# AlvinYH/Faster-VoxelPose

Hardware: AMD Instinct MI355X
Metric: frames/sec at 5-view 80x80x20 voxel (heatmaps -> 3D joints); MPJPE vs ref (mm) in mpjpe_vs_ref_mm (higher is better)
Workload: dtype f32

## Files before the change

faster-voxelpose_amd/csrc/fvp_project.hip:

```cpp
#include <hip/hip_runtime.h>

#include <cstdlib>

#include "fvp_common.h"
#include "fvp_geom.h"

namespace fvp {

template <int NV>
__global__ void __launch_bounds__(256) k_heat_to_cl(const float* __restrict__ heat, float* __restrict__ cl,
                                                    int J, int HW) {
  const int pix = blockIdx.x * 256 + threadIdx.x;
  const size_t bv = blockIdx.y;
  if (pix >= HW) return;
  const float* src = heat + bv * size_t(J) * HW + pix;
  float v[4 * NV];
#pragma unroll
  for (int j = 0; j < 4 * NV; ++j) v[j] = (j < J) ? src[size_t(j) * HW] : 0.0f;
  float4* dst = reinterpret_cast<float4*>(cl + (bv * HW + pix) * size_t(4 * NV));
#pragma unroll
  for (int q = 0; q < NV; ++q) dst[q] = make_float4(v[4 * q], v[4 * q + 1], v[4 * q + 2], v[4 * q + 3]);
}

__global__ void __launch_bounds__(256) k_sample_grid(const float* __restrict__ ax, const float* __restrict__ ay,
                                                     const float* __restrict__ az, int nx, int ny, int nz,
                                                     const Cam* __restrict__ cams, FvpGeom g,
                                                     float* __restrict__ grid) {
  const int n = nx * ny * nz;
  const int i = blockIdx.x * 256 + threadIdx.x;
  const int v = blockIdx.y;
  if (i >= n) return;
  const int iz = i % nz, iy = (i / nz) % ny, ix = i / (nz * ny);
  float gx, gy;
  project_norm(cams[v], g, ax[ix], ay[iy], az[iz], gx, gy);
  grid[(size_t(v) * n + i) * 2 + 0] = gx;
  grid[(size_t(v) * n + i) * 2 + 1] = gy;
}

template <int NV>
__device__ __forceinline__ void backproject_point(const float* __restrict__ heat_cl_frame,
                                                  const Cam* __restrict__ cams, const FvpGeom& g, float wx,
                                                  float wy, float wz, float (&acc)[4 * NV]) {
  const size_t view_stride = size_t(g.H) * g.W * (4 * NV);
  for (int v = 0; v < g.V; ++v) {
    float gx, gy;
    project_norm(cams[v], g, wx, wy, wz, gx, gy);
    const Taps t = bilinear_taps(gx, gy, g.W, g.H);
    float s[4 * NV];
    if (t.inside) {
      sample_view<NV>(heat_cl_frame + v * view_stride, t, s);
    } else {
#pragma unroll
      for (int c = 0; c < 4 * NV; ++c) s[c] = 0.0f;
    }
#pragma unroll
    for (int c = 0; c < 4 * NV; ++c) acc[c] = (v == 0) ? s[c] : __fadd_rn(acc[c], s[c]);
  }
  const float nv = float(g.V);
#pragma unroll
  for (int c = 0; c < 4 * NV; ++c) acc[c] = clampf(__fdiv_rn(acc[c], nv), 0.0f, 1.0f);
}

template <int NV>
__global__ void __launch_bounds__(256)
k_project_whole(const float* __restrict__ heat_cl, const Cam* __restrict__ cams, const int* __restrict__ frame_set,
                const float* __restrict__ ax, const float* __restrict__ ay, const float* __restrict__ az, int X,
                int Y, int Z, FvpGeom g, float* __restrict__ cubes, float* __restrict__ zmax) {
  __shared__ float sm[4 * NV][256];
  const int cpb = 256 / Z;
  const int b = blockIdx.y;
  const int t = threadIdx.x;
  const int cl_ = t / Z, z = t - cl_ * Z;
  const int col = blockIdx.x * cpb + cl_;
  const int ncol = X * Y;
  const bool active = cl_ < cpb && col < ncol;
  const int J = g.J;
  float acc[4 * NV];
#pragma unroll
  for (int c = 0; c < 4 * NV; ++c) acc[c] = 0.0f;
  if (active) {
    const int x = col / Y, y = col - x * Y;
    const float* frame = heat_cl + size_t(b) * g.V * g.H * g.W * (4 * NV);
    backproject_point<NV>(frame, cams + size_t(frame_set[b]) * g.V, g, ax[x], ay[y], az[z], acc);
    if (cubes) {
// ... 613 lines not shown
  if (nP == 0) return 0;
  ProfScope ps(FVP_K_OTHER, as_stream(s));
  const int per = (C * C + 255) / 256;
  const dim3 grid(J, nP);
  const size_t lds = size_t(C) * (C + 1) * sizeof(float);
#define FVP_TRIMAX(PER_) hipLaunchKernelGGL(k_triplane_max<PER_>, grid, dim3(256), lds, as_stream(s), cubes, planes, J, C)
  if (per <= 1) FVP_TRIMAX(1);
  else if (per <= 4) FVP_TRIMAX(4);
  else if (per <= 16) FVP_TRIMAX(16);
  else FVP_TRIMAX(64);
#undef FVP_TRIMAX
  return launch_status();
}

extern "C" int fvp_project_individual_triplane(const float* heat_cl, const float* cams, const int32_t* frame_set,
                                               const int32_t* person_frame, const uint8_t* person_valid,
                                               const int32_t* boxes, const float* fx, const float* fy,
                                               const float* fz, const int32_t* fine, int C, int nP, const FvpGeom* g,
                                               float* planes, int persons_per_frame, const float* fine_grid,
                                               fvp_stream_t s) {
  FVP_REQUIRE(heat_cl && cams && frame_set && person_frame && boxes && fx && fy && fz && planes && nP >= 0);
  FVP_REQUIRE(!fine_grid || fine);
  if (int e = check_geom(g)) return e;
  if (int e = check_cube(C)) return e;
  if (nP == 0) return 0;
  const int ppf = (persons_per_frame > 0 && nP % persons_per_frame == 0) ? persons_per_frame : nP;
  [[maybe_unused]] const int chunks = ceil_div(C * C, 256);
  const int nvl = ceil_div(g->JP, 16);
  ProfScope ps(FVP_K_PROJECT_TRIPLANE, as_stream(s));
  const int F0 = fine_grid ? fine[0] : 0, F1 = fine_grid ? fine[1] : 0, F2 = fine_grid ? fine[2] : 0;
  const int nby = ceil_div(C, kBY);
#if FVP_DIAG
  const int nbx = ceil_div(C, kBX);
  static const bool gather = fvp::diag_env("FVP_TRIPLANE_GATHER") != nullptr;
  const bool quad_form = fvp::diag_env("FVP_TRIPLANE_QUAD") != nullptr;
  static const int tri_ablate_env = fvp::diag_env("FVP_TRI_ABLATE") ? atoi(fvp::diag_env("FVP_TRI_ABLATE")) : 0;
  const char* tt_env = fvp::diag_env("FVP_TRI_TWO_TILE");
  const bool staged = fvp::diag_env("FVP_TRIPLANE_STAGED") != nullptr;
  const bool force_lane = fvp::diag_env("FVP_TRIPLANE_LANE") != nullptr;
  const bool lane_form = !gather && !quad_form && g->JP <= 20 && ((staged && g->JP != 16) || force_lane);
  const int tri_ablate = (tri_ablate_env & ~16) | ((tt_env ? atoi(tt_env) != 0 : lane_form) ? 16 : 0);
  auto cap_lim = [](int cap) { const char* e = fvp::diag_env("FVP_TRI_CAP_PX"); const int v = e ? atoi(e) : cap; return v > 0 && v < cap ? v : cap; };
  const int cap_px = int((36 * 1024) / (size_t(g->JP) * 4));
  const size_t lds = 2 * size_t(cap_px) * g->JP * 4 + 64;
  if (lane_form) {
    const int lq = (g->JP / 4) | 1;
    const int cap_px = int((36 * 1024) / (size_t(lq) * 16));
    const size_t lds = 2 * size_t(cap_px) * lq * 16 + 64;
    FVP_LIMIT(size_t(cap_px) * lq * 4 >= size_t(kBX * kBY + (kBX + kBY) * 32) * g->JP);
#define CALL2(NQ_, CACHED_)                                                                                       \
  {                                                                                                                \
    static LdsOptIn optin;                                                                                         \
    auto k = &k_project_triplane_lds2<NQ_, CACHED_>;                                                              \
    if (int e = lds_opt_in(optin, reinterpret_cast<const void*>(k), lds)) return e;                                \
    hipLaunchKernelGGL(k, dim3(nbx * nby * nP), dim3(kTriThreads), lds, as_stream(s), heat_cl,                     \
                       reinterpret_cast<const Cam*>(cams), frame_set, person_frame, person_valid, boxes, fx, fy, fz, C, \
                       nP, nbx, nby, ppf, cap_px, *g, fine_grid, F0, F1, F2, planes, tri_ablate, cap_lim(cap_px));                  \
  }
#define CASE2(NQ_) case NQ_: if (fine_grid) CALL2(NQ_, true) else CALL2(NQ_, false) break;
    switch (g->JP / 4) {
      CASE2(1) CASE2(2) CASE2(3) CASE2(4) CASE2(5)
      default: return FVP_ELIMIT;
    }
#undef CASE2
#undef CALL2
    return launch_status();
  }
  const bool blk_form = !gather && !quad_form && !staged;
#else
  constexpr bool blk_form = true;
#endif
  if (blk_form && nvl <= 2) {
    const int nbx2 = ceil_div(C, kBlkBX);
    const int bz = nvl == 2 ? 16 : kBlkBZ;
    int zsh = 0;
    while ((1 << zsh) < C) ++zsh;
    const size_t lds_z = (size_t(kBlkBX + kBY) << zsh) * (g->JP + 1) * 4;
#if FVP_DIAG
    const char* zr_env = fvp::diag_env("FVP_TRI_ZRES");
    const bool zres = zr_env && atoi(zr_env) != 0 && (1 << zsh) >= bz && lds_z <= kTriZresMaxLds;
#else
    constexpr bool zres = false;
#endif
    const size_t lds_b = zres ? lds_z : size_t(kBlkBX * kBY + (kBlkBX + kBY) * bz) * (g->JP + 1) * 4;
#define CALLB(NVL_, CACHED_, ZRES_)                                                                                          \
  hipLaunchKernelGGL((k_project_triplane_blk<NVL_, CACHED_, ZRES_>), dim3(nbx2 * nby * nP), dim3(kBlkThreads), lds_b,       \
                     as_stream(s), heat_cl, reinterpret_cast<const Cam*>(cams), frame_set, person_frame, person_valid, boxes, \
                     fx, fy, fz, C, nP, nbx2, nby, ppf, *g, fine_grid, F0, F1, F2, planes, zsh)
#if FVP_DIAG
#define CALLB2(NVL_)                                                                     \
  {                                                                                      \
    if (fine_grid) { if (zres) CALLB(NVL_, true, true); else CALLB(NVL_, true, false); } \
    else { if (zres) CALLB(NVL_, false, true); else CALLB(NVL_, false, false); }         \
  }
#else
#define CALLB2(NVL_)                                                                     \
  {                                                                                      \
    if (fine_grid) CALLB(NVL_, true, false); else CALLB(NVL_, false, false);             \
  }
#endif
    const bool q5 = nvl == 2 && g->JP == 20 && !zres && fvp::diag_env("FVP_TRI_NO_Q5") == nullptr;
    if (q5) {
      if (fine_grid)
        hipLaunchKernelGGL((k_project_triplane_blk<2, true, false, true>), dim3(nbx2 * nby * nP), dim3(kBlkThreads), lds_b, as_stream(s),
                           heat_cl, reinterpret_cast<const Cam*>(cams), frame_set, person_frame, person_valid, boxes, fx, fy, fz, C, nP,
                           nbx2, nby, ppf, *g, fine_grid, F0, F1, F2, planes, zsh);
      else
        hipLaunchKernelGGL((k_project_triplane_blk<2, false, false, true>), dim3(nbx2 * nby * nP), dim3(kBlkThreads), lds_b, as_stream(s),
                           heat_cl, reinterpret_cast<const Cam*>(cams), frame_set, person_frame, person_valid, boxes, fx, fy, fz, C, nP,
                           nbx2, nby, ppf, *g, fine_grid, F0, F1, F2, planes, zsh);
    } else if (nvl == 2) CALLB2(2) else CALLB2(1)
#undef CALLB2
#undef CALLB
    return launch_status();
  }
#if FVP_DIAG
  if (!gather && nvl <= 2) {
    FVP_LIMIT(cap_px >= kBX * kBY + (kBX + kBY) * (nvl == 1 ? 32 : 16));
#define CALL(NVL_, CACHED_)                                                                                        \
  {                                                                                                                \
    static LdsOptIn optin;                                                                                         \
    auto k = &k_project_triplane_lds<NVL_, CACHED_>;                                                               \
    if (int e = lds_opt_in(optin, reinterpret_cast<const void*>(k), lds)) return e;                                \
    hipLaunchKernelGGL(k, dim3(nbx * nby * nP), dim3(kTriThreads), lds, as_stream(s), heat_cl,                     \
                       reinterpret_cast<const Cam*>(cams), frame_set, person_frame, person_valid, boxes, fx, fy, fz, C, \
                       nP, nbx, nby, ppf, cap_px, *g, fine_grid, F0, F1, F2, planes, tri_ablate, cap_lim(cap_px));                  \
  }
    if (nvl == 1) {
      if (fine_grid) CALL(1, true) else CALL(1, false)
    } else {
      if (fine_grid) CALL(2, true) else CALL(2, false)
    }
#undef CALL
    return launch_status();
  }
  if (nvl == 1) {
    auto k = &k_project_triplane<1>;
    hipLaunchKernelGGL(k, dim3(chunks * nP), dim3(1024), 0, as_stream(s), heat_cl, reinterpret_cast<const Cam*>(cams),
                       frame_set, person_frame, person_valid, boxes, fx, fy, fz, C, nP, chunks, ppf, *g, planes);
  } else if (nvl == 2) {
    auto k = &k_project_triplane<2>;
    hipLaunchKernelGGL(k, dim3(chunks * nP), dim3(1024), 0, as_stream(s), heat_cl, reinterpret_cast<const Cam*>(cams),
                       frame_set, person_frame, person_valid, boxes, fx, fy, fz, C, nP, chunks, ppf, *g, planes);
  } else {
    return FVP_ELIMIT;
  }
  return launch_status();
#else
  return FVP_ELIMIT;
#endif
}
```

faster-voxelpose_amd/csrc/fvp_project_lds.h:

```cpp
#pragma once
#include <type_traits>
#include <climits>

namespace fvp {

typedef float f32x2 __attribute__((ext_vector_type(2)));
#ifndef FVP_TRI_PACKED
#define FVP_TRI_PACKED 1
#endif
#ifndef FVP_TRI_EXPLICIT_AS
#define FVP_TRI_EXPLICIT_AS 1
#endif

typedef float f32x4v __attribute__((ext_vector_type(4)));
__device__ __forceinline__ float4 lds_ld4(const float* p) {
  const f32x4v v = *(const __attribute__((address_space(3))) f32x4v*)p;
  return make_float4(v.x, v.y, v.z, v.w);
}
__device__ __forceinline__ float4 glb_ld4(const float* p) {
  const f32x4v v = *(const __attribute__((address_space(1))) f32x4v*)p;
  return make_float4(v.x, v.y, v.z, v.w);
}

struct TapL {
// ... 300 lines not shown
        }
      }
      if (rcur.big) {
        __syncthreads();
        if (v + 1 < V && rnxt.staged) issue_dma(v + 1, rnxt);
      }
      cur = nxt;
      rcur = rnxt;
    }
    __syncthreads();
    if (ablate & 4) continue;
    int* cxy = reinterpret_cast<int*>(smem);
    int* cxz = cxy + kBX * kBY * JP;
    int* cyz = cxz + kBX * BZ * JP;
    const int ncell = (kBX * kBY + (kBX + kBY) * BZ) * JP;
    for (int i = t; i < ncell; i += NT) cxy[i] = 0;
    __syncthreads();
#pragma unroll
    for (int n = 0; n < NVL; ++n)
#pragma unroll
      for (int c = 0; c < 4; ++c) {
        const int ch = 16 * n + 4 * q + c;
        float mz = 0.0f;
#pragma unroll
        for (int i = 0; i < VPT; ++i) {
          const float val = fmaxf(acc[i][n][c], 0.0f);
          mz = fmaxf(mz, val);
          if (val > 0.0f && ch < JP) {
            const int z = zs + 4 * i;
            atomicMax(&cxz[(xx * BZ + z) * JP + ch], __float_as_int(val));
            atomicMax(&cyz[(yy * BZ + z) * JP + ch], __float_as_int(val));
          }
        }
        int mi = __float_as_int(mz);
        mi = imax(mi, dpp_i<0x124>(mi));
        mi = imax(mi, dpp_i<0x128>(mi));
        if (zs == 0 && mi > 0 && ch < JP) cxy[(xx * kBY + yy) * JP + ch] = mi;
      }
    __syncthreads();
    const int lz0 = gz0 - tl2;
    for (int i = t; i < kBX * kBY * J; i += NT) {
      const int ch = i / (kBX * kBY), col = i - ch * (kBX * kBY), cx = col / kBY, cy = col - cx * kBY;
      const int raw = cxy[col * JP + ch];
      if (raw > 0 && gx0 + cx < e0 && gy0 + cy < e1) {
        const int vv = __float_as_int(clampf(__fdiv_rn(__int_as_float(raw), nv), 0.0f, 1.0f));
        if (vv > 0) plane_max(&pxy[size_t(ch) * CC + (gx0 + cx - tl0) * C + (gy0 + cy - tl1)], vv);
      }
    }
    for (int i = t; i < (kBX + kBY) * BZ * J; i += NT) {
      const int ch = i / ((kBX + kBY) * BZ), r = i - ch * ((kBX + kBY) * BZ), a = r / BZ, z = r - a * BZ;
      if (gz0 + z < e2) {
        const int raw = cxz[r * JP + ch];
        const int vv = raw > 0 ? __float_as_int(clampf(__fdiv_rn(__int_as_float(raw), nv), 0.0f, 1.0f)) : 0;
        if (vv > 0) {
          if (a < kBX) {
            if (gx0 + a < e0) plane_max(&pxz[size_t(ch) * CC + (gx0 + a - tl0) * C + lz0 + z], vv);
          } else if (gy0 + a - kBX < e1) {
            plane_max(&pyz[size_t(ch) * CC + (gy0 + a - kBX - tl1) * C + lz0 + z], vv);
          }
        }
      }
    }
    __syncthreads();
  }
}

#endif

#ifndef FVP_TRI_BLK_OCC
#define FVP_TRI_BLK_OCC 4
#endif
#ifndef FVP_TRI_BLK_BX
#define FVP_TRI_BLK_BX 4
#endif
#ifndef FVP_TRI_BLK_BZ
#define FVP_TRI_BLK_BZ 16
#endif
constexpr int kBlkBX = FVP_TRI_BLK_BX, kBlkBZ = FVP_TRI_BLK_BZ;
constexpr int kBlkThreads = kBlkBX * kBY * 4 * 4;
#ifndef FVP_TRI_ZRES_MAX_KB
#define FVP_TRI_ZRES_MAX_KB 48
#endif
constexpr size_t kTriZresMaxLds = size_t(FVP_TRI_ZRES_MAX_KB) * 1024;
template <int NVL, bool CACHED, bool ZRES, bool Q5 = false>
__global__ void __launch_bounds__(kBlkThreads, FVP_TRI_BLK_OCC)
k_project_triplane_blk(const float* __restrict__ heat_cl, const Cam* __restrict__ cams, const int* __restrict__ frame_set,
                       const int* __restrict__ person_frame, const uint8_t* __restrict__ person_valid,
                       const int* __restrict__ boxes, const float* __restrict__ fx, const float* __restrict__ fy,
                       const float* __restrict__ fz, int C, int nP, int nbx, int nby, int ppf, FvpGeom g,
                       const float* __restrict__ fgrid, int F0, int F1, int F2, float* __restrict__ planes, int zsh) {
  static_assert(!Q5 || (NVL == 2 && !ZRES), "the five-quad form replaces the two-group form of the per-z-block kernel");
  constexpr int NVA = Q5 ? 1 : NVL;
  constexpr int BZ = NVL == 1 ? kBlkBZ : 16;
  constexpr int VPT = BZ / 4;
  constexpr int OWN = VPT / 4;
  HIP_DYNAMIC_SHARED(float, smem)
  constexpr int NT = kBlkThreads;
  constexpr int kBX = kBlkBX;
  const int J = g.J, JP = g.JP, CC = C * C, V = g.V, W = g.W, H = g.H;
  int p, blk;
  {
    const int id = blockIdx.x;
    const int bpp = nbx * nby, bpf = ppf * bpp;
    const int nframes = nP / ppf;
    if (nframes % 8 == 0) {
      const int xcd = id & 7, j = id >> 3;
      const int frame = xcd + 8 * (j / bpf), r = j % bpf;
      p = frame * ppf + r / bpp;
      blk = r % bpp;
    } else {
      p = id / bpp;
      blk = id % bpp;
    }
  }
  if (person_valid && !person_valid[p]) return;
  const int* bx = boxes + p * 9;
  const int tl0 = bx[0], tl1 = bx[1], tl2 = bx[2];
  const int s0 = bx[3], s1 = bx[4], s2 = bx[5], e0 = bx[6], e1 = bx[7], e2 = bx[8];
  if (s0 >= e0 || s1 >= e1 || s2 >= e2) return;
  const int xb = blk / nby, yb = blk - xb * nby;
  const int gx0 = s0 + xb * kBX, gy0 = s1 + yb * kBY;
  if (gx0 >= e0 || gy0 >= e1) return;

  const int t = threadIdx.x, q = t & 3;
  const int slot = t >> 2, zs = slot & 3, yy = (slot >> 2) & (kBY - 1), xx = slot / (4 * kBY);
  const int gxi = gx0 + xx, gyi = gy0 + yy;
  const bool col_in = gxi < e0 && gyi < e1;
  const int b = person_frame[p];
  const size_t view_stride = size_t(H) * W * JP;
  const float* frame = heat_cl + size_t(b) * V * view_stride;
  const Cam* cm = cams + size_t(frame_set[b]) * V;
  const float wx = col_in ? fx[gxi] : 0.0f, wy = col_in ? fy[gyi] : 0.0f;
  const size_t nfine = size_t(F0) * F1 * F2;
  const float2* gcol = CACHED ? reinterpret_cast<const float2*>(fgrid) + size_t(frame_set[b]) * V * nfine +
                                    (size_t(col_in ? gxi : 0) * F1 + (col_in ? gyi : 0)) * F2
                              : nullptr;
  float* pxy = planes + (size_t(p) * 3 + 0) * J * CC;
  float* pxz = planes + (size_t(p) * 3 + 1) * J * CC;
  float* pyz = planes + (size_t(p) * 3 + 2) * J * CC;
  const float nv = float(V);
  const int JPp = JP + 1;
  [[maybe_unused]] int mxy[NVL][4];
  [[maybe_unused]] const int zt = 1 << zsh;
  if constexpr (ZRES) {
#pragma unroll
    for (int n = 0; n < NVL; ++n)
#pragma unroll
      for (int c = 0; c < 4; ++c) mxy[n][c] = 0;
    int* cz = reinterpret_cast<int*>(smem);
    const int ncell = ((kBX + kBY) << zsh) * JPp;
    for (int i = t; i < ncell; i += NT) cz[i] = 0;
    __syncthreads();
  }

  for (int gz0 = s2; gz0 < e2; gz0 += BZ) {
    float acc[VPT][NVA][4];
#pragma unroll
    for (int i = 0; i < VPT; ++i)
#pragma unroll
      for (int n = 0; n < NVA; ++n)
#pragma unroll
        for (int c = 0; c < 4; ++c) acc[i][n][c] = 0.0f;
    [[maybe_unused]] float accx[OWN][1][4];
#pragma unroll
    for (int kk = 0; kk < OWN; ++kk)
#pragma unroll
      for (int c = 0; c < 4; ++c) accx[kk][0][c] = 0.0f;
    float2 crd[OWN];
    auto load_coords = [&](int v) {
#pragma unroll
      for (int k = 0; k < OWN; ++k) {
        const int gzi = gz0 + zs + 4 * (q + 4 * k);
        crd[k] = gcol[size_t(v) * nfine + (gzi < F2 ? gzi : F2 - 1)];
      }
    };
    if (CACHED) load_coords(0);
    for (int v = 0; v < V; ++v) {
      TapL mine[OWN];
#pragma unroll
      for (int k = 0; k < OWN; ++k) {
        const int gzi = gz0 + zs + 4 * (q + 4 * k);
        const bool vin = col_in && gzi < e2;
        TapL d;
        d.base = d.dx = d.dy = 0;
        d.w[0] = d.w[1] = d.w[2] = d.w[3] = 0.0f;
        if (vin) {
          float sx, sy;
          if (CACHED) {
            sx = crd[k].x;
            sy = crd[k].y;
          } else {
            project_norm(cm[v], g, wx, wy, fz[gzi], sx, sy);
          }
          int x0, y0, inside;
          float w4[4];
          tap_origin(sx, sy, W, H, x0, y0, w4, inside);
          const int cx0 = imin(imax(x0, 0), W - 1), cx1 = imin(imax(x0 + 1, 0), W - 1);
          const int cy0 = imin(imax(y0, 0), H - 1), cy1 = imin(imax(y0 + 1, 0), H - 1);
          d.base = (cy0 * W + cx0) * JP;
          d.dx = (cx1 - cx0) * JP;
          d.dy = (cy1 - cy0) * W * JP;
#pragma unroll
          for (int c = 0; c < 4; ++c) d.w[c] = ((inside >> c) & 1) ? w4[c] : 0.0f;
        }
        mine[k] = d;
      }
      if (CACHED && v + 1 < V) load_coords(v + 1);
#ifdef FVP_TRI_BLK_NOSAMPLE
      if (mine[0].base != -12345) { acc[0][0][0] += mine[0].w[0] + mine[OWN - 1].w[3] + float(mine[0].base); continue; }
#endif
      const float* gsrc = frame + size_t(v) * view_stride;
      auto sample = [&](const TapL& tv, auto& a, auto own) {
        constexpr bool kOwn = decltype(own)::value;
#pragma unroll
        for (int n = 0; n < (kOwn ? 1 : NVA); ++n) {
          const int ch0 = kOwn ? 16 : 16 * n + 4 * q;
          if (kOwn || ch0 < JP) {
            const float* p0 = gsrc + tv.base + ch0;
            const float4 v0 = glb_ld4(p0), v1 = glb_ld4(p0 + tv.dx), v2 = glb_ld4(p0 + tv.dy), v3 = glb_ld4(p0 + tv.dy + tv.dx);
            const f32x2 w0 = f32x2{tv.w[0], tv.w[0]}, w1 = f32x2{tv.w[1], tv.w[1]}, w2 = f32x2{tv.w[2], tv.w[2]},
                        w3 = f32x2{tv.w[3], tv.w[3]};
            f32x2 lo = f32x2{v0.x, v0.y} * w0, hi = f32x2{v0.z, v0.w} * w0;
            lo = __builtin_elementwise_fma(f32x2{v1.x, v1.y}, w1, lo);
            hi = __builtin_elementwise_fma(f32x2{v1.z, v1.w}, w1, hi);
            lo = __builtin_elementwise_fma(f32x2{v2.x, v2.y}, w2, lo);
            hi = __builtin_elementwise_fma(f32x2{v2.z, v2.w}, w2, hi);
            lo = __builtin_elementwise_fma(f32x2{v3.x, v3.y}, w3, lo);
            hi = __builtin_elementwise_fma(f32x2{v3.z, v3.w}, w3, hi);
            const f32x2 alo = f32x2{a[n][0], a[n][1]} + lo, ahi = f32x2{a[n][2], a[n][3]} + hi;
            a[n][0] = alo.x; a[n][1] = alo.y; a[n][2] = ahi.x; a[n][3] = ahi.y;
          }
        }
      };
#pragma unroll
      for (int k = 0; k < OWN; ++k) {
        { const TapL tv = quad_bcast_l<0>(mine[k]); sample(tv, acc[4 * k + 0], std::false_type{}); }
        { const TapL tv = quad_bcast_l<1>(mine[k]); sample(tv, acc[4 * k + 1], std::false_type{}); }
        { const TapL tv = quad_bcast_l<2>(mine[k]); sample(tv, acc[4 * k + 2], std::false_type{}); }
        { const TapL tv = quad_bcast_l<3>(mine[k]); sample(tv, acc[4 * k + 3], std::false_type{}); }
        if constexpr (Q5) sample(mine[k], accx[k], std::true_type{});
      }
    }
#ifdef FVP_TRI_BLK_NOMAX
    if (acc[0][0][0] != 1.2345e-30f) continue;
#endif
    if constexpr (ZRES) {
      int* rxz = reinterpret_cast<int*>(smem);
      int* ryz = rxz + ((kBX << zsh) * JPp);
      const int zb = gz0 - s2 + zs;
#pragma unroll
      for (int n = 0; n < NVL; ++n)
#pragma unroll
        for (int c = 0; c < 4; ++c) {
          const int ch = 16 * n + 4 * q + c;
          float mz = 0.0f;
#pragma unroll
          for (int i = 0; i < VPT; ++i) {
            const float val = fmaxf(acc[i][n][c], 0.0f);
            mz = fmaxf(mz, val);
            if (val > 0.0f && ch < JP) {
              const int z = zb + 4 * i;
              atomicMax(&rxz[((xx << zsh) + z) * JPp + ch], __float_as_int(val));
              atomicMax(&ryz[((yy << zsh) + z) * JPp + ch], __float_as_int(val));
            }
          }
          int mi = __float_as_int(mz);
          mi = imax(mi, dpp_i<0x124>(mi));
          mi = imax(mi, dpp_i<0x128>(mi));
          mxy[n][c] = imax(mxy[n][c], mi);
        }
      continue;
    }
    int* cxy = reinterpret_cast<int*>(smem);
    int* cxz = cxy + kBX * kBY * JPp;
    int* cyz = cxz + kBX * BZ * JPp;
    const int ncell = (kBX * kBY + (kBX + kBY) * BZ) * JPp;
    __syncthreads();
    for (int i = t; i < ncell; i += NT) cxy[i] = 0;
    __syncthreads();
#pragma unroll
    for (int n = 0; n < NVA; ++n)
#pragma unroll
      for (int c = 0; c < 4; ++c) {
        const int ch = 16 * n + 4 * q + c;
        float mz = 0.0f;
#pragma unroll
        for (int i = 0; i < VPT; ++i) {
          const float val = fmaxf(acc[i][n][c], 0.0f);
          mz = fmaxf(mz, val);
          if (val > 0.0f && ch < JP) {
            const int z = zs + 4 * i;
            atomicMax(&cxz[(xx * BZ + z) * JPp + ch], __float_as_int(val));
            atomicMax(&cyz[(yy * BZ + z) * JPp + ch], __float_as_int(val));
          }
        }
        int mi = __float_as_int(mz);
        mi = imax(mi, dpp_i<0x124>(mi));
        mi = imax(mi, dpp_i<0x128>(mi));
        if (zs == 0 && mi > 0 && ch < JP) cxy[(xx * kBY + yy) * JPp + ch] = mi;
      }
    if constexpr (Q5) {
#pragma unroll
      for (int c = 0; c < 4; ++c) {
        const int ch = 16 + c;
        float mz = 0.0f;
#pragma unroll
        for (int kk = 0; kk < OWN; ++kk) {
          const float val = fmaxf(accx[kk][0][c], 0.0f);
          mz = fmaxf(mz, val);
          if (val > 0.0f) {
            const int z = zs + 4 * (4 * kk + q);
            atomicMax(&cxz[(xx * BZ + z) * JPp + ch], __float_as_int(val));
            atomicMax(&cyz[(yy * BZ + z) * JPp + ch], __float_as_int(val));
          }
        }
        int mi = __float_as_int(mz);
        mi = imax(mi, dpp_i<0x121>(mi));
        mi = imax(mi, dpp_i<0x122>(mi));
        mi = imax(mi, dpp_i<0x124>(mi));
        mi = imax(mi, dpp_i<0x128>(mi));
        if (zs == 0 && q == 0 && mi > 0) cxy[(xx * kBY + yy) * JPp + ch] = mi;
      }
    }
    __syncthreads();
    const int lz0 = gz0 - tl2;
    for (int i = t; i < kBX * kBY * J; i += NT) {
      const int ch = i / (kBX * kBY), col = i - ch * (kBX * kBY), cx = col / kBY, cy = col - cx * kBY;
      const int raw = cxy[col * JPp + ch];
      if (raw > 0 && gx0 + cx < e0 && gy0 + cy < e1) {
        const int vv = __float_as_int(clampf(__fdiv_rn(__int_as_float(raw), nv), 0.0f, 1.0f));
        if (vv > 0) plane_max(&pxy[size_t(ch) * CC + (gx0 + cx - tl0) * C + (gy0 + cy - tl1)], vv);
      }
    }
    for (int i = t; i < (kBX + kBY) * BZ * J; i += NT) {
      const int ch = i / ((kBX + kBY) * BZ), r = i - ch * ((kBX + kBY) * BZ), a = r / BZ, z = r - a * BZ;
      if (gz0 + z < e2) {
        const int raw = cxz[r * JPp + ch];
        const int vv = raw > 0 ? __float_as_int(clampf(__fdiv_rn(__int_as_float(raw), nv), 0.0f, 1.0f)) : 0;
        if (vv > 0) {
          if (a < kBX) {
            if (gx0 + a < e0) plane_max(&pxz[size_t(ch) * CC + (gx0 + a - tl0) * C + lz0 + z], vv);
          } else if (gy0 + a - kBX < e1) {
            plane_max(&pyz[size_t(ch) * CC + (gy0 + a - kBX - tl1) * C + lz0 + z], vv);
          }
        }
      }
    }
  }
  if constexpr (ZRES) {
    __syncthreads();
    if (zs == 0 && col_in) {
#pragma unroll
      for (int n = 0; n < NVL; ++n)
#pragma unroll
        for (int c = 0; c < 4; ++c) {
          const int ch = 16 * n + 4 * q + c;
          if (ch < J && mxy[n][c] > 0) {
            const int vv = __float_as_int(clampf(__fdiv_rn(__int_as_float(mxy[n][c]), nv), 0.0f, 1.0f));
            if (vv > 0) plane_max(&pxy[size_t(ch) * CC + (gxi - tl0) * C + (gyi - tl1)], vv);
          }
        }
    }
    const int* cz = reinterpret_cast<const int*>(smem);
    const int nz = e2 - s2, lz0 = s2 - tl2;
    const int rows = (kBX + kBY) << zsh;
    for (int i = t; i < rows * J; i += NT) {
      static_assert(kBX + kBY == 8, "row count is a power of two");
      const int ch = i >> (zsh + 3), r = i & (rows - 1), a = r >> zsh, z = r & (zt - 1);
      if (z < nz) {
        const int raw = cz[r * JPp + ch];
        const int vv = raw > 0 ? __float_as_int(clampf(__fdiv_rn(__int_as_float(raw), nv), 0.0f, 1.0f)) : 0;
        if (vv > 0) {
          if (a < kBX) {
            if (gx0 + a < e0) plane_max(&pxz[size_t(ch) * CC + (gx0 + a - tl0) * C + lz0 + z], vv);
          } else if (gy0 + a - kBX < e1) {
            plane_max(&pyz[size_t(ch) * CC + (gy0 + a - kBX - tl1) * C + lz0 + z], vv);
          }
        }
      }
    }
  }
}

#if FVP_DIAG
template <int NQ, bool CACHED>
__global__ void __launch_bounds__(kTriThreads, 4)
k_project_triplane_lds2(const float* __restrict__ heat_cl, const Cam* __restrict__ cams, const int* __restrict__ frame_set,
                        const int* __restrict__ person_frame, const uint8_t* __restrict__ person_valid,
                        const int* __restrict__ boxes, const float* __restrict__ fx, const float* __restrict__ fy,
                        const float* __restrict__ fz, int C, int nP, int nbx, int nby, int ppf, int cap_px, FvpGeom g,
                        const float* __restrict__ fgrid, int F0, int F1, int F2, float* __restrict__ planes, int ablate, int cap_lim) {
  constexpr int BZ = 32, VPT = 2, JP = 4 * NQ;
  constexpr int LQ = NQ | 1, LP = 4 * LQ;
  HIP_DYNAMIC_SHARED(float, smem)
  constexpr int NT = kTriThreads;
  const int J = g.J, CC = C * C, V = g.V, W = g.W, H = g.H;
  const int tile_sz = cap_px * LP;
  int* rect = reinterpret_cast<int*>(smem + 2 * size_t(tile_sz));
  int p, blk;
  {
    const int id = blockIdx.x;
    const int bpp = nbx * nby, bpf = ppf * bpp;
    const int nframes = nP / ppf;
    if (nframes % 8 == 0) {
      const int xcd = id & 7, j = id >> 3;
      const int frame = xcd + 8 * (j / bpf), r = j % bpf;
      p = frame * ppf + r / bpp;
      blk = r % bpp;
    } else {
      p = id / bpp;
      blk = id % bpp;
    }
  }
  if (person_valid && !person_valid[p]) return;
  const int* bx = boxes + p * 9;
  const int tl0 = bx[0], tl1 = bx[1], tl2 = bx[2];
  const int s0 = bx[3], s1 = bx[4], s2 = bx[5], e0 = bx[6], e1 = bx[7], e2 = bx[8];
  if (s0 >= e0 || s1 >= e1 || s2 >= e2) return;
  const int xb = blk / nby, yb = blk - xb * nby;
  const int gx0 = s0 + xb * kBX, gy0 = s1 + yb * kBY;
  if (gx0 >= e0 || gy0 >= e1) return;

  const int t = threadIdx.x, lane = t & 63, wave = t >> 6;
  const int z16 = t & 15, yy = (t >> 4) & (kBY - 1), xx = t >> 6;
  const int gxi = gx0 + xx, gyi = gy0 + yy;
  const bool col_in = gxi < e0 && gyi < e1;
  const int b = person_frame[p];
  const size_t view_stride = size_t(H) * W * JP;
  const float* frame = heat_cl + size_t(b) * V * view_stride;
  const Cam* cm = cams + size_t(frame_set[b]) * V;
  const float wx = col_in ? fx[gxi] : 0.0f, wy = col_in ? fy[gyi] : 0.0f;
  const size_t nfine = size_t(F0) * F1 * F2;
  const float2* gcol = CACHED ? reinterpret_cast<const float2*>(fgrid) + size_t(frame_set[b]) * V * nfine +
                                    (size_t(col_in ? gxi : 0) * F1 + (col_in ? gyi : 0)) * F2
                              : nullptr;
  float* pxy = planes + (size_t(p) * 3 + 0) * J * CC;
  float* pxz = planes + (size_t(p) * 3 + 1) * J * CC;
  float* pyz = planes + (size_t(p) * 3 + 2) * J * CC;
  const float nv = float(V);

  struct Own { int xy[VPT]; int inside[VPT]; float w[VPT][4]; };
  float2 crd[VPT];
  auto load_coords = [&](int v, int gz0) {
#pragma unroll
    for (int k = 0; k < VPT; ++k) {
      const int gzi = gz0 + z16 + 16 * k;
      crd[k] = gcol[size_t(v) * nfine + (gzi < F2 ? gzi : F2 - 1)];
    }
  };
  auto project = [&](int v, int gz0, Own& o) {
    int mnx = INT_MIN, mxx = INT_MIN, mny = INT_MIN, mxy = INT_MIN;
#pragma unroll
    for (int k = 0; k < VPT; ++k) {
      const int gzi = gz0 + z16 + 16 * k;
      const bool vin = col_in && gzi < e2;
      o.inside[k] = 0;
      o.xy[k] = 0;
      o.w[k][0] = o.w[k][1] = o.w[k][2] = o.w[k][3] = 0.0f;
      if (vin) {
// ... 199 lines not shown
```

Baseline: 3038.

## Group y-blocks per workgroup and accumulate xz/xy plane maxima in LDS across them

Each workgroup in the triplane projection kernel now walks several y-tiles (ygrp) over a bounded z-span, instead of owning a single x/y tile. The xz-plane partial maxima stay in LDS across the y loop and are flushed once. The yz plane is double-buffered by parity so the zeroing barrier between z-blocks goes away, and when a workgroup owns a cell outright it writes it with a plain store instead of an atomic max. This is meant to cut per-block LDS clearing, barriers and global atomicMax traffic on the planes, in exchange for fewer workgroups and more complex indexing.

```diff
diff --git a/faster-voxelpose_amd/csrc/fvp_project.hip b/faster-voxelpose_amd/csrc/fvp_project.hip
--- a/faster-voxelpose_amd/csrc/fvp_project.hip
+++ b/faster-voxelpose_amd/csrc/fvp_project.hip
@@ -1,5 +1,6 @@
 #include <hip/hip_runtime.h>
 
+#include <algorithm>
 #include <cstdlib>
 
 #include "fvp_common.h"
@@ -779,11 +780,19 @@
 #else
     constexpr bool zres = false;
 #endif
-    const size_t lds_b = zres ? lds_z : size_t(kBlkBX * kBY + (kBlkBX + kBY) * bz) * (g->JP + 1) * 4;
+    int ygrp = kTriYGrp;
+#if FVP_DIAG
+    if (const char* yg_env = fvp::diag_env("FVP_TRI_YGRP")) ygrp = atoi(yg_env);
+#endif
+    ygrp = zres ? 1 : std::min(std::max(ygrp, 1), nby);
+    const int zspsh = zres ? zsh : std::min(zsh, kTriZSpanSh);
+    const int nzs = 1 << (zsh - zspsh);
+    const int nwg = nbx2 * ceil_div(nby, ygrp) * nzs * nP;
+    const size_t lds_b = zres ? lds_z : size_t((kBlkBX << zspsh) + 2 * kBY * bz + kBlkBX * kBY) * (g->JP + 1) * 4;
 #define CALLB(NVL_, CACHED_, ZRES_)                                                                                          \
-  hipLaunchKernelGGL((k_project_triplane_blk<NVL_, CACHED_, ZRES_>), dim3(nbx2 * nby * nP), dim3(kBlkThreads), lds_b,       \
+  hipLaunchKernelGGL((k_project_triplane_blk<NVL_, CACHED_, ZRES_>), dim3(nwg), dim3(kBlkThreads), lds_b,                   \
                      as_stream(s), heat_cl, reinterpret_cast<const Cam*>(cams), frame_set, person_frame, person_valid, boxes, \
-                     fx, fy, fz, C, nP, nbx2, nby, ppf, *g, fine_grid, F0, F1, F2, planes, zsh)
+                     fx, fy, fz, C, nP, nbx2, nby, ppf, *g, fine_grid, F0, F1, F2, planes, zsh, ygrp, nzs, zspsh)
 #if FVP_DIAG
 #define CALLB2(NVL_)                                                                     \
   {                                                                                      \
@@ -799,13 +808,13 @@
     const bool q5 = nvl == 2 && g->JP == 20 && !zres && fvp::diag_env("FVP_TRI_NO_Q5") == nullptr;
     if (q5) {
       if (fine_grid)
-        hipLaunchKernelGGL((k_project_triplane_blk<2, true, false, true>), dim3(nbx2 * nby * nP), dim3(kBlkThreads), lds_b, as_stream(s),
+        hipLaunchKernelGGL((k_project_triplane_blk<2, true, false, true>), dim3(nwg), dim3(kBlkThreads), lds_b, as_stream(s),
                            heat_cl, reinterpret_cast<const Cam*>(cams), frame_set, person_frame, person_valid, boxes, fx, fy, fz, C, nP,
-                           nbx2, nby, ppf, *g, fine_grid, F0, F1, F2, planes, zsh);
+                           nbx2, nby, ppf, *g, fine_grid, F0, F1, F2, planes, zsh, ygrp, nzs, zspsh);
       else
-        hipLaunchKernelGGL((k_project_triplane_blk<2, false, false, true>), dim3(nbx2 * nby * nP), dim3(kBlkThreads), lds_b, as_stream(s),
+        hipLaunchKernelGGL((k_project_triplane_blk<2, false, false, true>), dim3(nwg), dim3(kBlkThreads), lds_b, as_stream(s),
                            heat_cl, reinterpret_cast<const Cam*>(cams), frame_set, person_frame, person_valid, boxes, fx, fy, fz, C, nP,
-                           nbx2, nby, ppf, *g, fine_grid, F0, F1, F2, planes, zsh);
+                           nbx2, nby, ppf, *g, fine_grid, F0, F1, F2, planes, zsh, ygrp, nzs, zspsh);
     } else if (nvl == 2) CALLB2(2) else CALLB2(1)
 #undef CALLB2
 #undef CALLB
diff --git a/faster-voxelpose_amd/csrc/fvp_project_lds.h b/faster-voxelpose_amd/csrc/fvp_project_lds.h
--- a/faster-voxelpose_amd/csrc/fvp_project_lds.h
+++ b/faster-voxelpose_amd/csrc/fvp_project_lds.h
@@ -406,13 +406,19 @@
 #define FVP_TRI_ZRES_MAX_KB 48
 #endif
 constexpr size_t kTriZresMaxLds = size_t(FVP_TRI_ZRES_MAX_KB) * 1024;
+#ifndef FVP_TRI_YGRP
+#define FVP_TRI_YGRP 4
+#endif
+constexpr int kTriYGrp = FVP_TRI_YGRP;
+constexpr int kTriZSpanSh = 6;
 template <int NVL, bool CACHED, bool ZRES, bool Q5 = false>
 __global__ void __launch_bounds__(kBlkThreads, FVP_TRI_BLK_OCC)
 k_project_triplane_blk(const float* __restrict__ heat_cl, const Cam* __restrict__ cams, const int* __restrict__ frame_set,
                        const int* __restrict__ person_frame, const uint8_t* __restrict__ person_valid,
                        const int* __restrict__ boxes, const float* __restrict__ fx, const float* __restrict__ fy,
                        const float* __restrict__ fz, int C, int nP, int nbx, int nby, int ppf, FvpGeom g,
-                       const float* __restrict__ fgrid, int F0, int F1, int F2, float* __restrict__ planes, int zsh) {
+                       const float* __restrict__ fgrid, int F0, int F1, int F2, float* __restrict__ planes, int zsh,
+                       int ygrp, int nzs, int zspsh) {
   static_assert(!Q5 || (NVL == 2 && !ZRES), "the five-quad form replaces the two-group form of the per-z-block kernel");
   constexpr int NVA = Q5 ? 1 : NVL;
   constexpr int BZ = NVL == 1 ? kBlkBZ : 16;
@@ -422,10 +428,11 @@
   constexpr int NT = kBlkThreads;
   constexpr int kBX = kBlkBX;
   const int J = g.J, JP = g.JP, CC = C * C, V = g.V, W = g.W, H = g.H;
+  const int nyg = (nby + ygrp - 1) / ygrp;
   int p, blk;
   {
     const int id = blockIdx.x;
-    const int bpp = nbx * nby, bpf = ppf * bpp;
+    const int bpp = nbx * nyg * nzs, bpf = ppf * bpp;
     const int nframes = nP / ppf;
     if (nframes % 8 == 0) {
       const int xcd = id & 7, j = id >> 3;
@@ -439,45 +446,65 @@
   }
   if (person_valid && !person_valid[p]) return;
   const int* bx = boxes + p * 9;
-  const int tl0 = bx[0], tl1 = bx[1], tl2 = bx[2];
+  int tl0 = bx[0], tl1 = bx[1], tl2 = bx[2];
   const int s0 = bx[3], s1 = bx[4], s2 = bx[5], e0 = bx[6], e1 = bx[7], e2 = bx[8];
   if (s0 >= e0 || s1 >= e1 || s2 >= e2) return;
-  const int xb = blk / nby, yb = blk - xb * nby;
-  const int gx0 = s0 + xb * kBX, gy0 = s1 + yb * kBY;
-  if (gx0 >= e0 || gy0 >= e1) return;
+  if constexpr (NVL == 2 && !CACHED) {
+    FVP_OPAQUE_V(tl0); FVP_OPAQUE_V(tl1); FVP_OPAQUE_V(tl2);
+  }
+  const int xb = blk / (nyg * nzs), yz = blk - xb * (nyg * nzs), yg = yz / nzs, zsp = yz - yg * nzs;
+  const int zspan = 1 << zspsh;
+  const int gx0 = s0 + xb * kBX;
+  const int yb0 = yg * ygrp, yb1 = imin(yb0 + ygrp, nby);
+  const int zs0 = s2 + zsp * zspan, ze = imin(e2, zs0 + zspan);
+  if (gx0 >= e0 || s1 + yb0 * kBY >= e1 || zs0 >= e2) return;
+  const int gyend = imin(e1, s1 + yb1 * kBY);
+  const bool xy_shared = ZRES || nzs > 1;
+  const bool xz_shared = nyg > 1;
 
   const int t = threadIdx.x, q = t & 3;
   const int slot = t >> 2, zs = slot & 3, yy = (slot >> 2) & (kBY - 1), xx = slot / (4 * kBY);
-  const int gxi = gx0 + xx, gyi = gy0 + yy;
-  const bool col_in = gxi < e0 && gyi < e1;
+  const int gxi = gx0 + xx;
   const int b = person_frame[p];
   const size_t view_stride = size_t(H) * W * JP;
   const float* frame = heat_cl + size_t(b) * V * view_stride;
   const Cam* cm = cams + size_t(frame_set[b]) * V;
-  const float wx = col_in ? fx[gxi] : 0.0f, wy = col_in ? fy[gyi] : 0.0f;
   const size_t nfine = size_t(F0) * F1 * F2;
+  float* const pp = planes + size_t(p) * 3 * J * CC;
+  const float nv = float(V);
+  const int JPp = JP + 1;
+  [[maybe_unused]] const int zt = 1 << zsh;
+  constexpr bool XYREG = NVL == 1 || ZRES;
+  constexpr int kYzRows = kBY * BZ;
+  int* const oxz = reinterpret_cast<int*>(smem);
+  int* const oyz = oxz + (kBX << zspsh) * JPp;
+  [[maybe_unused]] int* const oxy = oyz + 2 * kYzRows * JPp + (xx * kBY + yy) * JPp;
+  const float wx = gxi < e0 ? fx[gxi] : 0.0f;
+  if constexpr (ZRES) {
+    int* cz = reinterpret_cast<int*>(smem);
+    const int ncell = ((kBX + kBY) << zsh) * JPp;
+    for (int i = t; i < ncell; i += NT) cz[i] = 0;
+  } else {
+    const int ncell = ((kBX << zspsh) + 2 * kYzRows + (XYREG ? 0 : kBX * kBY)) * JPp;
+    for (int i = t; i < ncell; i += NT) oxz[i] = 0;
+  }
+  __syncthreads();
+  [[maybe_unused]] int par = 0;
+
+  for (int gy0 = s1 + yb0 * kBY; gy0 < gyend; gy0 += kBY) {
+  const int gyi = gy0 + yy;
+  const bool col_in = gxi < e0 && gyi < e1;
+  const float wy = col_in ? fy[gyi] : 0.0f;
   const float2* gcol = CACHED ? reinterpret_cast<const float2*>(fgrid) + size_t(frame_set[b]) * V * nfine +
                                     (size_t(col_in ? gxi : 0) * F1 + (col_in ? gyi : 0)) * F2
                               : nullptr;
-  float* pxy = planes + (size_t(p) * 3 + 0) * J * CC;
-  float* pxz = planes + (size_t(p) * 3 + 1) * J * CC;
-  float* pyz = planes + (size_t(p) * 3 + 2) * J * CC;
-  const float nv = float(V);
-  const int JPp = JP + 1;
-  [[maybe_unused]] int mxy[NVL][4];
-  [[maybe_unused]] const int zt = 1 << zsh;
-  if constexpr (ZRES) {
-#pragma unroll
-    for (int n = 0; n < NVL; ++n)
-#pragma unroll
-      for (int c = 0; c < 4; ++c) mxy[n][c] = 0;
-    int* cz = reinterpret_cast<int*>(smem);
-    const int ncell = ((kBX + kBY) << zsh) * JPp;
-    for (int i = t; i < ncell; i += NT) cz[i] = 0;
-    __syncthreads();
-  }
-
-  for (int gz0 = s2; gz0 < e2; gz0 += BZ) {
+  [[maybe_unused]] int mxy[NVA][4];
+#pragma unroll
+  for (int n = 0; n < NVA; ++n)
+#pragma unroll
+    for (int c = 0; c < 4; ++c) mxy[n][c] = 0;
+
+  for (int gz0 = zs0; gz0 < ze; gz0 += BZ) {
     float acc[VPT][NVA][4];
 #pragma unroll
     for (int i = 0; i < VPT; ++i)
@@ -504,7 +531,7 @@
 #pragma unroll
       for (int k = 0; k < OWN; ++k) {
         const int gzi = gz0 + zs + 4 * (q + 4 * k);
-        const bool vin = col_in && gzi < e2;
+        const bool vin = col_in && gzi < ze;
         TapL d;
         d.base = d.dx = d.dy = 0;
         d.w[0] = d.w[1] = d.w[2] = d.w[3] = 0.0f;
@@ -568,40 +595,12 @@
 #ifdef FVP_TRI_BLK_NOMAX
     if (acc[0][0][0] != 1.2345e-30f) continue;
 #endif
-    if constexpr (ZRES) {
-      int* rxz = reinterpret_cast<int*>(smem);
-      int* ryz = rxz + ((kBX << zsh) * JPp);
-      const int zb = gz0 - s2 + zs;
-#pragma unroll
-      for (int n = 0; n < NVL; ++n)
-#pragma unroll
-        for (int c = 0; c < 4; ++c) {
-          const int ch = 16 * n + 4 * q + c;
-          float mz = 0.0f;
-#pragma unroll
-          for (int i = 0; i < VPT; ++i) {
-            const float val = fmaxf(acc[i][n][c], 0.0f);
-            mz = fmaxf(mz, val);
-            if (val > 0.0f && ch < JP) {
-              const int z = zb + 4 * i;
-              atomicMax(&rxz[((xx << zsh) + z) * JPp + ch], __float_as_int(val));
-              atomicMax(&ryz[((yy << zsh) + z) * JPp + ch], __float_as_int(val));
-            }
-          }
-          int mi = __float_as_int(mz);
-          mi = imax(mi, dpp_i<0x124>(mi));
-          mi = imax(mi, dpp_i<0x128>(mi));
-          mxy[n][c] = imax(mxy[n][c], mi);
-        }
-      continue;
-    }
-    int* cxy = reinterpret_cast<int*>(smem);
-    int* cxz = cxy + kBX * kBY * JPp;
-    int* cyz = cxz + kBX * BZ * JPp;
-    const int ncell = (kBX * kBY + (kBX + kBY) * BZ) * JPp;
-    __syncthreads();
-    for (int i = t; i < ncell; i += NT) cxy[i] = 0;
-    __syncthreads();
+    int aP = JP + 1, aJ = J;
+    FVP_OPAQUE(aP); FVP_OPAQUE(aJ);
+    int* const rxz = ZRES ? reinterpret_cast<int*>(smem) + ((xx << zsh) + (gz0 - s2)) * aP
+                          : oxz + ((xx << zspsh) + (gz0 - zs0)) * aP;
+    int* const ryz = ZRES ? reinterpret_cast<int*>(smem) + ((kBX << zsh) + (yy << zsh) + (gz0 - s2)) * aP
+                          : oyz + (par * kYzRows + yy * BZ) * aP;
 #pragma unroll
     for (int n = 0; n < NVA; ++n)
 #pragma unroll
@@ -612,16 +611,17 @@
         for (int i = 0; i < VPT; ++i) {
           const float val = fmaxf(acc[i][n][c], 0.0f);
           mz = fmaxf(mz, val);
-          if (val > 0.0f && ch < JP) {
+          if (val > 0.0f && ch < aJ) {
             const int z = zs + 4 * i;
-            atomicMax(&cxz[(xx * BZ + z) * JPp + ch], __float_as_int(val));
-            atomicMax(&cyz[(yy * BZ + z) * JPp + ch], __float_as_int(val));
+            atomicMax(&rxz[z * aP + ch], __float_as_int(val));
+            atomicMax(&ryz[z * aP + ch], __float_as_int(val));
           }
         }
         int mi = __float_as_int(mz);
         mi = imax(mi, dpp_i<0x124>(mi));
         mi = imax(mi, dpp_i<0x128>(mi));
-        if (zs == 0 && mi > 0 && ch < JP) cxy[(xx * kBY + yy) * JPp + ch] = mi;
+        if constexpr (XYREG) mxy[n][c] = imax(mxy[n][c], mi);
+        else if (zs == 0 && ch < aJ && mi > 0) atomicMax(&oxy[ch], mi);
       }
     if constexpr (Q5) {
 #pragma unroll
@@ -632,10 +632,10 @@
         for (int kk = 0; kk < OWN; ++kk) {
           const float val = fmaxf(accx[kk][0][c], 0.0f);
           mz = fmaxf(mz, val);
-          if (val > 0.0f) {
+          if (val > 0.0f && ch < aJ) {
             const int z = zs + 4 * (4 * kk + q);
-            atomicMax(&cxz[(xx * BZ + z) * JPp + ch], __float_as_int(val));
-            atomicMax(&cyz[(yy * BZ + z) * JPp + ch], __float_as_int(val));
+            atomicMax(&rxz[z * aP + ch], __float_as_int(val));
+            atomicMax(&ryz[z * aP + ch], __float_as_int(val));
           }
         }
         int mi = __float_as_int(mz);
@@ -643,48 +643,62 @@
         mi = imax(mi, dpp_i<0x122>(mi));
         mi = imax(mi, dpp_i<0x124>(mi));
         mi = imax(mi, dpp_i<0x128>(mi));
-        if (zs == 0 && q == 0 && mi > 0) cxy[(xx * kBY + yy) * JPp + ch] = mi;
-      }
-    }
-    __syncthreads();
-    const int lz0 = gz0 - tl2;
-    for (int i = t; i < kBX * kBY * J; i += NT) {
-      const int ch = i / (kBX * kBY), col = i - ch * (kBX * kBY), cx = col / kBY, cy = col - cx * kBY;
-      const int raw = cxy[col * JPp + ch];
-      if (raw > 0 && gx0 + cx < e0 && gy0 + cy < e1) {
-        const int vv = __float_as_int(clampf(__fdiv_rn(__int_as_float(raw), nv), 0.0f, 1.0f));
-        if (vv > 0) plane_max(&pxy[size_t(ch) * CC + (gx0 + cx - tl0) * C + (gy0 + cy - tl1)], vv);
-      }
-    }
-    for (int i = t; i < (kBX + kBY) * BZ * J; i += NT) {
-      const int ch = i / ((kBX + kBY) * BZ), r = i - ch * ((kBX + kBY) * BZ), a = r / BZ, z = r - a * BZ;
-      if (gz0 + z < e2) {
-        const int raw = cxz[r * JPp + ch];
-        const int vv = raw > 0 ? __float_as_int(clampf(__fdiv_rn(__int_as_float(raw), nv), 0.0f, 1.0f)) : 0;
-        if (vv > 0) {
-          if (a < kBX) {
-            if (gx0 + a < e0) plane_max(&pxz[size_t(ch) * CC + (gx0 + a - tl0) * C + lz0 + z], vv);
-          } else if (gy0 + a - kBX < e1) {
-            plane_max(&pyz[size_t(ch) * CC + (gy0 + a - kBX - tl1) * C + lz0 + z], vv);
-          }
-        }
+        if (zs == 0 && q == 0 && ch < aJ && mi > 0) atomicMax(&oxy[ch], mi);
+      }
+    }
+    if constexpr (!ZRES) {
+      __syncthreads();
+      int mJ = J, mC = C, mP = JPp;
+      FVP_OPAQUE(mJ); FVP_OPAQUE(mC); FVP_OPAQUE(mP);
+      int* const cyz = oyz + par * kYzRows * mP;
+      const int lz0 = gz0 - tl2;
+      for (int i = t; i < kYzRows * mJ; i += NT) {
+        const int ch = i / kYzRows, r = i - ch * kYzRows, a = r / BZ, z = r - a * BZ;
+        const int raw = cyz[r * mP + ch];
+        if (raw > 0) {
+          cyz[r * mP + ch] = 0;
+          const int vv = __float_as_int(clampf(__fdiv_rn(__int_as_float(raw), nv), 0.0f, 1.0f));
+          if (vv > 0 && gz0 + z < ze && gy0 + a < e1)
+            plane_max(&pp[size_t(2 * mJ + ch) * (mC * mC) + (gy0 + a - tl1) * mC + lz0 + z], vv);
+        }
+      }
+      par ^= 1;
+    }
+  }
+  if (zs == 0 && col_in) {
+    int mJ = J, mC = C;
+    FVP_OPAQUE(mJ); FVP_OPAQUE(mC);
+    float* const cell = pp + (gxi - tl0) * mC + (gyi - tl1);
+    const bool shared = xy_shared;
+    auto put = [&](int ch, int raw) {
+      if constexpr (!XYREG) {
+        raw = ch < mJ ? oxy[ch] : 0;
+        if (raw > 0) oxy[ch] = 0;
+      }
+      if (ch < mJ && raw > 0) {
+        const float val = clampf(__fdiv_rn(__int_as_float(raw), nv), 0.0f, 1.0f);
+        if (val > 0.0f) {
+          if (shared) plane_max(&cell[size_t(ch) * (mC * mC)], __float_as_int(val));
+          else cell[size_t(ch) * (mC * mC)] = val;
+        }
+      }
+    };
+#pragma unroll
+    for (int n = 0; n < NVA; ++n)
+#pragma unroll
+      for (int c = 0; c < 4; ++c) {
+        if constexpr (XYREG) put(16 * n + 4 * q + c, mxy[n][c]);
+        else put(16 * n + 4 * q + c, 0);
+      }
+    if constexpr (Q5) {
+      if (q == 0) {
+#pragma unroll
+        for (int c = 0; c < 4; ++c) put(16 + c, 0);
       }
     }
   }
   if constexpr (ZRES) {
     __syncthreads();
-    if (zs == 0 && col_in) {
-#pragma unroll
-      for (int n = 0; n < NVL; ++n)
-#pragma unroll
-        for (int c = 0; c < 4; ++c) {
-          const int ch = 16 * n + 4 * q + c;
-          if (ch < J && mxy[n][c] > 0) {
-            const int vv = __float_as_int(clampf(__fdiv_rn(__int_as_float(mxy[n][c]), nv), 0.0f, 1.0f));
-            if (vv > 0) plane_max(&pxy[size_t(ch) * CC + (gxi - tl0) * C + (gyi - tl1)], vv);
-          }
-        }
-    }
     const int* cz = reinterpret_cast<const int*>(smem);
     const int nz = e2 - s2, lz0 = s2 - tl2;
     const int rows = (kBX + kBY) << zsh;
@@ -696,9 +710,31 @@
         const int vv = raw > 0 ? __float_as_int(clampf(__fdiv_rn(__int_as_float(raw), nv), 0.0f, 1.0f)) : 0;
         if (vv > 0) {
           if (a < kBX) {
-            if (gx0 + a < e0) plane_max(&pxz[size_t(ch) * CC + (gx0 + a - tl0) * C + lz0 + z], vv);
+            if (gx0 + a < e0) plane_max(&pp[size_t(J + ch) * CC + (gx0 + a - tl0) * C + lz0 + z], vv);
           } else if (gy0 + a - kBX < e1) {
-            plane_max(&pyz[size_t(ch) * CC + (gy0 + a - kBX - tl1) * C + lz0 + z], vv);
+            plane_max(&pp[size_t(2 * J + ch) * CC + (gy0 + a - kBX - tl1) * C + lz0 + z], vv);
+          }
+        }
+      }
+    }
+  }
+  }
+  if constexpr (!ZRES) {
+    __syncthreads();
+    int mJ = J, mC = C, mP = JPp, mS = zspsh;
+    FVP_OPAQUE(mJ); FVP_OPAQUE(mC); FVP_OPAQUE(mP); FVP_OPAQUE(mS);
+    const int rows = kBX << mS, nz = ze - zs0, lz0 = zs0 - tl2;
+    const bool shared = xz_shared;
+    for (int i = t; i < rows * mJ; i += NT) {
+      const int ch = i / rows, r = i - ch * rows, a = r >> mS, z = r & ((1 << mS) - 1);
+      if (z < nz && gx0 + a < e0) {
+        const int raw = oxz[r * mP + ch];
+        if (raw > 0) {
+          const float val = clampf(__fdiv_rn(__int_as_float(raw), nv), 0.0f, 1.0f);
+          float* const cell = &pp[size_t(mJ + ch) * (mC * mC) + (gx0 + a - tl0) * mC + lz0 + z];
+          if (val > 0.0f) {
+            if (shared) plane_max(cell, __float_as_int(val));
+            else *cell = val;
           }
         }
       }
```

Result: slower. 2907 (-4.3%).
